# simonfuhrmann/mve

Measured on NVIDIA H100. Metric: mvs_depth_pixels_per_second, higher is better.
Workload: dtype f32

## Files before the change

### mve_b200/csrc/b200mvs.cu

```cuda
#include "../../include/b200mvs.h"
#include "patch_opt.cuh"
#include "patch_warp.cuh"
#include "patch_thread.cuh"
#include "pset_device.cuh"
#include "device_buffer.cuh"

#include <algorithm>
#include <cmath>
#include <cstdarg>
#include <cstddef>
#include <cstdio>
#include <cstring>
#include <cstdlib>
#include <functional>
#include <map>
#include <chrono>
#include <ctime>
#include <mutex>
#include <string>
#include <thread>
#include <atomic>
#include <vector>

using namespace b200mvs;
// ... 43 lines not shown

struct Entry {
    int xy;
    int jobdir;
    float conf, depth, dzI, dzJ;
    unsigned slots;
    int pad;
};
static_assert(sizeof(Entry) == 32, "Entry layout");

__host__ __device__ __forceinline__ int pack_xy(int x, int y) { return x | (y << 16); }
__host__ __device__ __forceinline__ Entry make_entry(int xy, int job, int dir, float conf, float depth, float dzI, float dzJ, unsigned slots)
{
    return Entry{xy, job | (dir << 24), conf, depth, dzI, dzJ, slots, 0};
}
__device__ __forceinline__ int entry_x(const Entry& e) { return e.xy & 0xFFFF; }
__device__ __forceinline__ int entry_y(const Entry& e) { return (e.xy >> 16) & 0xFFFF; }
__device__ __forceinline__ int entry_job(const Entry& e) { return e.jobdir & 0xFFFFFF; }
__device__ __forceinline__ int entry_dir(const Entry& e) { return (e.jobdir >> 24) & 7; }
__device__ __forceinline__ int pixel_of(const JobParams& J, const Entry& e) { return entry_y(e) * J.W + entry_x(e); }
__device__ __forceinline__ long long tile_of(const JobParams& J, const Entry& e) { return J.tile_base + (long long)(entry_y(e) >> 4) * J.tiles_x + (entry_x(e) >> 4); }
__device__ __forceinline__ Entry child_entry(int xy, int job, int dir, const PatchOut& r) { return make_entry(xy, job, dir, r.conf, r.depth, r.dzI, r.dzJ, r.slots); }
__device__ __forceinline__ unsigned long long seed_key(float c, size_t i) { return ((unsigned long long)__float_as_uint(c) << 32) | (0xFFFFFFFFu - (unsigned)i); }

enum Counter { C_RUN = 0, C_NEXT = 1, C_OVERFLOW = 2, C_SETS = 3, C_OPTS = 4, C_SEED_OK = 5, C_FILLED = 6, C_TICKET = 7, C_NUM = 8 };

constexpr int HIST_FINE = 8192;
constexpr int HIST_COARSE = 64;
constexpr int HIST_PER_JOB = HIST_FINE + HIST_COARSE;
constexpr int DEFER_BIT = 1 << 27;
enum Phase { PH_SEED = 0, PH_SELECT = 1, PH_THRESHOLD = 2, PH_PICK = 3, PH_OPT = 4, PH_COMMIT = 5, PH_EXPAND = 6, PH_SORT = 7, PH_OPT_THREAD = 8, PH_NUM = 9 };
enum Stop { ST_RUN = 0, ST_CANCELLED = 2, ST_OVERFLOW = 3, ST_GROW = 4 };

struct FrontierCtl {
    unsigned long long bar;
    unsigned long long nlist[2];
    unsigned long long nrun;
    unsigned long long ticket;
    unsigned long long ticket2;
    unsigned long long sort_cursor;
    unsigned long long small_cursor;
    unsigned long long rounds, peak, barriers;
    unsigned long long ns[PH_NUM];
    unsigned long long need;
    unsigned long long resume_ncur, resume_nrun;
    int resume_p, resume_sorted;
    int stop;
    int pad;
};

struct HostMirror {
    volatile int cancel;
    volatile int pad;
    volatile unsigned long long round, queue;
};

constexpr int MAX_GROUP_VIEWS = 4000;

struct HostCounters {
    unsigned long long count[C_NUM + MAX_GROUP_VIEWS];
    FrontierCtl ctl;
};
static_assert(offsetof(HostCounters, ctl) >= sizeof(unsigned long long) * (C_NUM + MAX_GROUP_VIEWS),
              "the counters of a full group end before the control block");

cudaError_t dev_alloc(b200mvs_ctx* ctx, void** p, size_t bytes);
void dev_free(b200mvs_ctx* ctx, void* p, size_t bytes);

template <typename T> struct DevBuf {
    T* p = nullptr;
    size_t cap = 0;
    cudaError_t reserve(b200mvs_ctx* ctx, size_t n)
    {
        if (n <= cap) return cudaSuccess;
// ... 505 lines not shown
}

__host__ __device__ inline int slots_to_ids(const int* gview, int n_global, unsigned word, int32_t ids[4])
{
    int n = 0;
#pragma unroll
    for (int k = 0; k < 4; ++k) {
        const unsigned sl = (word >> (8 * k)) & 0xFF;
        ids[k] = sl < (unsigned)n_global ? gview[sl] : -1;
        n += ids[k] >= 0;
    }
    return n;
}

__global__ void k_slots_to_ids(const JobParams job, int32_t* __restrict__ out, bool aligned16)
{
    const size_t p = (size_t)blockIdx.x * blockDim.x + threadIdx.x;
    if (p >= (size_t)job.W * job.H) return;
    int32_t ids[4];
    slots_to_ids(job.gview, job.n_global, __ldg(job.slots + p), ids);
    int32_t* o = out + 4 * p;
    if (aligned16) *reinterpret_cast<int4*>(o) = make_int4(ids[0], ids[1], ids[2], ids[3]);
    else { o[0] = ids[0]; o[1] = ids[1]; o[2] = ids[2]; o[3] = ids[3]; }
}

#ifndef OPT_MIN_BLOCKS
#define OPT_MIN_BLOCKS 1
#endif
constexpr int OPT_WARPS = OPT_TPB / 32;
using PatchT = b200mvs::PatchW;
using PatchT1 = b200mvs::PatchT;
constexpr size_t OPT_LUT_BYTES = sizeof(float) * (256 * LUT_STRIDE);
constexpr size_t OPT_SMEM_BYTES = OPT_LUT_BYTES + (size_t)OPT_TPB * sizeof(PatchT1) + PatchT1::MT_BYTES;
static_assert(OPT_SMEM_BYTES + 8 + 1024 <= 196 * 1024, "the patch kernels' shared memory must stay within the 196 KB carve-out");
__device__ __forceinline__ PatchT1& thread_patch(float* smem)
{
    return reinterpret_cast<PatchT1*>(reinterpret_cast<unsigned char*>(smem) + OPT_LUT_BYTES)[threadIdx.x];
}

__device__ __forceinline__ Entry load_entry(const Entry* p)
{
    const int4 a = __ldcg(reinterpret_cast<const int4*>(p));
    const int4 b = __ldcg(reinterpret_cast<const int4*>(p) + 1);
    Entry e;
    e.xy = a.x; e.jobdir = a.y; e.conf = __int_as_float(a.z); e.depth = __int_as_float(a.w);
    e.dzI = __int_as_float(b.x); e.dzJ = __int_as_float(b.y); e.slots = (unsigned)b.z; e.pad = b.w;
    return e;
}

__device__ __forceinline__ PatchIn patch_in(const Entry& e)
{
    PatchIn pi;
    pi.x = entry_x(e); pi.y = entry_y(e);
    pi.depth = e.depth; pi.dzI = e.dzI; pi.dzJ = e.dzJ; pi.slots = e.slots;
    return pi;
}

__device__ __forceinline__ unsigned long long global_timer_ns()
{
    unsigned long long t;
    asm volatile("mov.u64 %0, %%globaltimer;" : "=l"(t));
    return t;
}

__device__ __forceinline__ void optimise_entries(PatchT& p, const Entry* list, PatchOut* res, unsigned long long n,
                                                 unsigned long long* ticket, const JobParams* jobs, unsigned long long* counters)
{
// ... 34 lines not shown
            base = __shfl_sync(act, base, leader);
            const unsigned long long w = base + (unsigned long long)__popc(act & ((1u << lane) - 1u));
            if (w >= n) break;
            idx = w;
            const Entry e = load_entry(&list[w]);
            p.begin(&jobs[entry_job(e)], patch_in(e));
            have = true;
            ++opts;
        }
        if (p.step()) {
            PatchOut po;
            p.finish(po);
            res[idx] = po;
            have = false;
        }
    }
    if (opts) {
        atomicAdd(&counters[C_SETS], (unsigned long long)p.n_sets);
        atomicAdd(&counters[C_OPTS], (unsigned long long)opts);
        p.n_sets = 0u;
    }
}

#ifndef OPT_THREAD_MIN
#define OPT_THREAD_MIN 8192
#endif

__global__ void __launch_bounds__(OPT_TPB, OPT_MIN_BLOCKS)
k_optimize(const Entry* __restrict__ in, PatchOut* __restrict__ out, int n, int mode,
           const DevSettings* __restrict__ st, const JobParams* __restrict__ jobs, const ViewParams* __restrict__ views,
           const float* __restrict__ g_lut, unsigned long long* counters)
{
    extern __shared__ float smem[];
    for (int i = threadIdx.x; i < 256 * LUT_STRIDE; i += blockDim.x) smem[i] = g_lut[i / LUT_STRIDE];
    __syncthreads();
    if (mode == 2 || (mode == 0 && n >= OPT_THREAD_MIN)) {
        PatchT1& p = thread_patch(smem);
        bind_thread(p, st, views, smem, (int)threadIdx.x);
        optimise_entries_t(p, in, out, (unsigned long long)n, &counters[C_TICKET], jobs, counters);
    } else {
        PatchT p;
        bind_thread(p, st, views, smem, (int)threadIdx.x);
        optimise_entries(p, in, out, (unsigned long long)n, &counters[C_TICKET], jobs, counters);
    }
}

__device__ __forceinline__ unsigned long long entry_key(const Entry& e)
{
    return ((unsigned long long)__float_as_uint(e.conf) << 8) | (unsigned long long)(7 - entry_dir(e));
}

struct FrontierParams {
    Entry* list[2];
    Entry* run;
    Entry* run2;
    unsigned* tile_cnt;
    unsigned long long* tile_off;
    long long n_tiles;
    PatchOut* res;
    unsigned char* written;
    unsigned long long cap;
    int n_seeds, n_jobs;
    const DevSettings* st;
    const JobParams* jobs;
    const ViewParams* views;
    const float* lut;
    unsigned long long* counters;
    FrontierCtl* ctl;
    unsigned* hist;
    int* thr_bin;
    HostMirror* host;
    volatile unsigned long long* host_filled;
    volatile int* host_cancel_job;
    int* job_cancel;
    long long thread_min;
    unsigned long long* job_run;
    int band_bins;
    int topk;
    int first_list;
};

__device__ __forceinline__ unsigned long long ld_relaxed_u64(const unsigned long long* p)
{
    unsigned long long v;
    asm volatile("ld.relaxed.gpu.global.u64 %0, [%1];" : "=l"(v) : "l"(p) : "memory");
    return v;
}
__device__ __forceinline__ void grid_barrier(unsigned long long* bar)
{
    __syncthreads();
    if (threadIdx.x == 0) {
        __threadfence();
        const unsigned long long nb = gridDim.x;
        const unsigned long long t = atomicAdd(bar, 1ull);
        const unsigned long long target = (t / nb + 1ull) * nb;
        while (ld_relaxed_u64(bar) < target) __nanosleep(64);
        __threadfence();
    }
    __syncthreads();
}
__device__ __forceinline__ int conf_bin(float c)
{
    const int b = (int)(c * (float)HIST_FINE);
    return b < 0 ? 0 : (b > HIST_FINE - 1 ? HIST_FINE - 1 : b);
}
__device__ __forceinline__ PatchOut load_result(const PatchOut* p)
{
    static_assert(sizeof(PatchOut) == 40, "PatchOut layout");
    const int2* q = reinterpret_cast<const int2*>(p);
    const int2 a = __ldcg(q), b = __ldcg(q + 1), c = __ldcg(q + 2), d = __ldcg(q + 3), e = __ldcg(q + 4);
    PatchOut r;
    r.conf = __int_as_float(a.x); r.depth = __int_as_float(a.y); r.dzI = __int_as_float(b.x); r.dzJ = __int_as_float(b.y);
    r.nx = __int_as_float(c.x); r.ny = __int_as_float(c.y); r.nz = __int_as_float(d.x); r.slots = (unsigned)d.y;
    r.iterations = e.x; r.flags = e.y;
    return r;
}
__device__ __forceinline__ unsigned long long take_slot(unsigned long long* counter)
{
    const unsigned m = __activemask();
    const int lane = threadIdx.x & 31, leader = __ffs(m) - 1;
    unsigned long long base = 0ull;
    if (lane == leader) base = atomicAdd(counter, (unsigned long long)__popc(m));
    base = __shfl_sync(m, base, leader);
    return base + (unsigned long long)__popc(m & ((1u << lane) - 1u));
}
__device__ __forceinline__ void count_for_job(unsigned long long* per_job, int j)
{
    const unsigned m = __match_any_sync(__activemask(), j);
    if ((int)(threadIdx.x & 31) == __ffs(m) - 1) atomicAdd(&per_job[j], (unsigned long long)__popc(m));
}
__device__ __forceinline__ void push_entry(const FrontierParams& P, int q, const Entry& o)
{
    const unsigned long long pos = take_slot(&P.ctl->nlist[q]);
// ... 68 lines not shown
        const PatchOut r = load_result(&P.res[i]);
        const int j = entry_job(e);
        const JobParams& J = P.jobs[j];
        const int x = entry_x(e), y = entry_y(e);
        const int nx[4] = {x - 1, x + 1, x, x};
        const int ny[4] = {y, y, y - 1, y + 1};
#pragma unroll
        for (int d = 0; d < 4; ++d) {
            const float c = __ldcg(&J.conf[ny[d] * J.W + nx[d]]);
            if (c < r.conf - 0.05f || c == 0.f) push_entry(P, 1 - p, child_entry(pack_xy(nx[d], ny[d]), j, d, r));
        }
    }
}

__device__ __forceinline__ bool end_round(FrontierCtl* ctl, unsigned long long n_cur, const HostMirror* host)
{
    ctl->rounds += 1ull;
    if (n_cur > ctl->peak) ctl->peak = n_cur;
    return host->cancel != 0;
}

__global__ void k_frontier_resume(const FrontierParams P)
{
    FrontierCtl* const ctl = P.ctl;
    const size_t gtid = (size_t)blockIdx.x * blockDim.x + threadIdx.x, gthreads = (size_t)gridDim.x * blockDim.x;
    push_neighbours(P, ctl->resume_p, ctl->resume_sorted ? P.run2 : P.run, ctl->resume_nrun, gtid, gthreads);
    if (gtid == 0) ctl->stop = end_round(ctl, ctl->resume_ncur, P.host) ? ST_CANCELLED : ST_RUN;
}

__global__ void __launch_bounds__(OPT_TPB, OPT_MIN_BLOCKS)
k_frontier(const FrontierParams P)
{
    extern __shared__ float smem[];
    for (int i = threadIdx.x; i < 256 * LUT_STRIDE; i += blockDim.x) smem[i] = P.lut[i / LUT_STRIDE];
    __syncthreads();
    const int lane = threadIdx.x & 31;
    const size_t gtid = (size_t)blockIdx.x * blockDim.x + threadIdx.x, gthreads = (size_t)gridDim.x * blockDim.x;
    FrontierCtl* const ctl = P.ctl;
    unsigned long long* const cnt = P.counters;
    unsigned long long* const filled = cnt + C_NUM;
    const bool lead = blockIdx.x == 0 && threadIdx.x == 0;
    const bool thresholded = P.band_bins > 0 || P.topk > 0;
    unsigned long long t_prev = lead ? global_timer_ns() : 0ull;
    unsigned long long n_bar = 0ull;
#define PHASE_END(ph) do { grid_barrier(&ctl->bar); ++n_bar; if (lead) { const unsigned long long t_ = global_timer_ns(); ctl->ns[ph] += t_ - t_prev; t_prev = t_; } } while (0)

    int p = P.first_list;
    bool seed_round = P.n_seeds > 0;
    for (;;) {
        unsigned long long n_cur = seed_round ? (unsigned long long)P.n_seeds : __ldcg(&ctl->nlist[p]);
        if (n_cur > P.cap) n_cur = P.cap;
        if (__ldcg(&ctl->stop) != ST_RUN || n_cur == 0ull) break;
        unsigned long long n_run = n_cur;
        if (!seed_round) {
        Entry* const cur = P.list[p];
        if (blockIdx.x == 0) {
            if (threadIdx.x == 0) { P.host->round = ctl->rounds; P.host->queue = n_cur; }
            for (int j = threadIdx.x; j < P.n_jobs; j += blockDim.x) {
                P.host_filled[j] = __ldcg(&filled[j]);
                if (P.host_cancel_job[j]) P.job_cancel[j] = 1;
            }
        }
        for (size_t i = gtid; i < n_cur; i += gthreads) {
            const Entry e = load_entry(&cur[i]);
            const int j = entry_job(e);
            const JobParams& J = P.jobs[j];
            const int idx = pixel_of(J, e);
// ... 35 lines not shown
                count_for_job(P.job_run, entry_job(e));
            } else
                push_entry(P, 1 - p, e);
        }
        if (thresholded)
            for (size_t i = gtid; i < (size_t)P.n_jobs * HIST_PER_JOB; i += gthreads) P.hist[i] = 0u;
        PHASE_END(PH_PICK);
        n_run = __ldcg(&ctl->nrun);
        if (lead) { ctl->nlist[p] = 0ull; ctl->need = 0ull; }
        }
        unsigned long long n_thread = 0ull;
        const Entry* run_cur = P.run;
        if (!seed_round && P.n_tiles > 0) {
            __shared__ unsigned long long s_big;
            if (threadIdx.x == 0) s_big = 0ull;
            __syncthreads();
            unsigned long long mine = 0ull;
            for (int j = threadIdx.x; j < P.n_jobs; j += blockDim.x) {
                const unsigned long long c = __ldcg(&P.job_run[j]);
                if (c >= (unsigned long long)P.thread_min) mine += c;
            }
            if (mine) atomicAdd(&s_big, mine);
            __syncthreads();
            n_thread = s_big;
        }
        if (n_thread > 0ull) {
            for (size_t i = gtid; i < n_run; i += gthreads) {
                const Entry e = load_entry(&P.run[i]);
                const int j = entry_job(e);
                if (__ldcg(&P.job_run[j]) < (unsigned long long)P.thread_min) continue;
                atomicAdd(&P.tile_cnt[tile_of(P.jobs[j], e)], 1u);
            }
            PHASE_END(PH_SORT);
            for (size_t b = gtid; b < (size_t)P.n_tiles; b += gthreads) {
                const unsigned c = __ldcg(&P.tile_cnt[b]);
                if (c) P.tile_off[b] = atomicAdd(&ctl->sort_cursor, (unsigned long long)c);
            }
            PHASE_END(PH_SORT);
            for (size_t i = gtid; i < n_run; i += gthreads) {
                const Entry e = load_entry(&P.run[i]);
                const int j = entry_job(e);
                if (__ldcg(&P.job_run[j]) < (unsigned long long)P.thread_min) {
                    P.run2[n_thread + take_slot(&ctl->small_cursor)] = e;
                    continue;
                }
                const long long bin = tile_of(P.jobs[j], e);
                const unsigned k = atomicSub(&P.tile_cnt[bin], 1u) - 1u;
                P.run2[__ldcg(&P.tile_off[bin]) + k] = e;
            }
            PHASE_END(PH_SORT);
            run_cur = P.run2;
        }
        const bool by_thread = n_thread > 0ull;
        if (by_thread) {
            PatchT1& pt = thread_patch(smem);
            bind_thread(pt, P.st, P.views, smem, (int)threadIdx.x);
            optimise_entries_t(pt, run_cur, P.res, n_thread, &ctl->ticket, P.jobs, cnt);
            __syncwarp();
        }
        if (n_run > n_thread) {
            PatchT pg;
            bind_thread(pg, P.st, P.views, smem, (int)threadIdx.x);
            optimise_entries(pg, run_cur + n_thread, P.res + n_thread, n_run - n_thread, by_thread ? &ctl->ticket2 : &ctl->ticket, P.jobs, cnt);
        }
        if (seed_round) {
            PHASE_END(PH_SEED);
            for (size_t i = gtid; i < (size_t)P.n_seeds; i += gthreads) {
                const float c = __ldcg(&P.res[i].conf);
                if (!(c > 0.f)) continue;
// ... 11 lines not shown
                const JobParams& J = P.jobs[j];
                const int idx = pixel_of(J, e);
                if (__ldcg(&J.sel[idx]) != seed_key(c, i)) continue;
                J.sel[idx] = 0ull;
                count_for_job(filled, j);
                const PatchOut r = load_result(&P.res[i]);
                write_pixel(J, idx, r);
                push_entry(P, 0, child_entry(e.xy, j, 4, r));
            }
            if (lead) ctl->ticket = 0ull;
            PHASE_END(PH_COMMIT);
            seed_round = false;
            p = 0;
            continue;
        }
        if (by_thread) PHASE_END(PH_OPT_THREAD); else PHASE_END(PH_OPT);
        for (size_t i = gtid; i < n_run; i += gthreads) {
            const Entry e = load_entry(&run_cur[i]);
            const PatchOut r = load_result(&P.res[i]);
            const int j = entry_job(e);
            const JobParams& J = P.jobs[j];
            const int idx = pixel_of(J, e);
            unsigned char w = 0;
            if (!(r.conf == 0.f)) {
                const float old = __ldcg(&J.conf[idx]);
                if (old <= 0.f) count_for_job(filled, j);
                if (old < r.conf) { write_pixel(J, idx, r); w = 1; }
            }
            P.written[i] = w;
            const unsigned act = __activemask(), wm = __ballot_sync(act, w);
            if (wm && lane == __ffs(act) - 1) atomicAdd(&ctl->need, 4ull * (unsigned long long)__popc(wm));
        }
        if (lead) {
            ctl->nrun = 0ull; ctl->ticket = 0ull; ctl->ticket2 = 0ull; ctl->sort_cursor = 0ull; ctl->small_cursor = 0ull;
            atomicAdd(&ctl->need, __ldcg(&ctl->nlist[1 - p]));
        }
        if (blockIdx.x == 0) for (int j = threadIdx.x; j < P.n_jobs; j += blockDim.x) P.job_run[j] = 0ull;
        PHASE_END(PH_COMMIT);
        if (__ldcg(&ctl->need) > P.cap) {
            if (lead) {
                ctl->resume_p = p; ctl->resume_ncur = n_cur; ctl->resume_nrun = n_run; ctl->resume_sorted = run_cur == P.run2;
                ctl->stop = ST_GROW;
            }
            break;
        }
        push_neighbours(P, p, run_cur, n_run, gtid, gthreads);
        if (lead) {
            if (end_round(ctl, n_cur, P.host)) ctl->stop = ST_CANCELLED;
            else if (__ldcg(&cnt[C_OVERFLOW])) ctl->stop = ST_OVERFLOW;
        }
        PHASE_END(PH_EXPAND);
        p ^= 1;
    }
    if (lead) ctl->barriers += n_bar;
    if (blockIdx.x == 0) {
        if (threadIdx.x == 0) { P.host->round = ctl->rounds; P.host->queue = 0ull; }
        for (int j = threadIdx.x; j < P.n_jobs; j += blockDim.x) P.host_filled[j] = __ldcg(&filled[j]);
    }
#undef PHASE_END
}

int require_device(const b200mvs_ctx* ctx)
{
    return ctx->device != B200MVS_DEVICE_NONE ? 0 : fail(B200MVS_ERR_CUDA, "planning context (B200MVS_DEVICE_NONE): no CUDA device, b200mvs has no CPU fallback");
}

int check_camera_args(const b200mvs_ctx* ctx, const char* fn, int id, bool image, int w, int h, const float* pp, const float* rot, const float* trans)
// ... 116 lines not shown
    std::memset(hp.data(), 0, hp.size() * sizeof(ViewParams));
    for (size_t i = 0; i < ctx->views.size(); ++i) {
        const HostView& v = ctx->views[i];
        ViewParams& p = hp[i];
        p.valid = v.valid ? 1 : 0;
        if (!v.valid) continue;
        std::memcpy(p.campos, v.campos, 12);
        std::memcpy(p.w2c, v.w2c, 48);
        std::memcpy(p.rot, v.rot, 36);
        p.inv_ax0 = v.lv[0].invproj[0];
        p.nlevels = (int)v.lv.size();
        for (size_t l = 0; l < v.lv.size(); ++l) {
            const HostLevel& L = v.lv[l];
            p.lv[l].ax = L.proj[0]; p.lv[l].ay = L.proj[4]; p.lv[l].cx = L.proj[2]; p.lv[l].cy = L.proj[5];
            p.lv[l].w = L.w; p.lv[l].h = L.h; p.lv[l].pitch = L.pitch; p.lv[l].img = v.has_image ? L.d_img : nullptr;
            p.lv[l].quad = v.has_image ? L.d_quad : nullptr;
        }
    }
    CK(cudaMemcpyAsync(ctx->d_views, hp.data(), hp.size() * sizeof(ViewParams), cudaMemcpyHostToDevice, ctx->stream));
    CK(cudaStreamSynchronize(ctx->stream));
    ctx->views_dirty = false;
    return 0;
}

cudaEvent_t get_event(b200mvs_ctx* ctx, size_t i)
{
    while (ctx->ev_pool.size() <= i) { cudaEvent_t e; cudaEventCreate(&e); ctx->ev_pool.push_back(e); }
    return ctx->ev_pool[i];
}

int prepare_kernels(b200mvs_ctx* ctx)
{
    if (ctx->frontier_grid) return 0;
    CK(cudaFuncSetAttribute(k_frontier, cudaFuncAttributeMaxDynamicSharedMemorySize, (int)OPT_SMEM_BYTES));
    CK(cudaFuncSetAttribute(k_optimize, cudaFuncAttributeMaxDynamicSharedMemorySize, (int)OPT_SMEM_BYTES));
    int per_sm = 0, per_sm_opt = 0, sms = 0;
    CK(cudaOccupancyMaxActiveBlocksPerMultiprocessor(&per_sm, k_frontier, OPT_TPB, OPT_SMEM_BYTES));
    CK(cudaOccupancyMaxActiveBlocksPerMultiprocessor(&per_sm_opt, k_optimize, OPT_TPB, OPT_SMEM_BYTES));
    CK(cudaDeviceGetAttribute(&sms, cudaDevAttrMultiProcessorCount, ctx->device));
    if (per_sm < 1 || per_sm_opt < 1) return fail(B200MVS_ERR_CUDA, "patch-optimisation kernels do not fit on an SM");
    ctx->optimize_grid = per_sm_opt * sms;
    ctx->frontier_grid = per_sm * sms;
    return 0;
}

JobParams make_job(const b200mvs_ctx* ctx, const b200mvs_settings& s, int ref, const std::vector<int>& gsel)
{
    const HostLevel& L = ctx->views[ref].lv[s.scale];
    JobParams J;
    std::memset(&J, 0, sizeof(J));
    J.ref_view = ref; J.W = L.w; J.H = L.h; J.n_global = (int)gsel.size();
    for (size_t k = 0; k < gsel.size(); ++k) J.gview[k] = gsel[k];
    J.ki0 = L.invproj[0]; J.ki2 = L.invproj[2]; J.ki4 = L.invproj[4]; J.ki5 = L.invproj[5];
    J.ref_img = L.d_img; J.ref_pitch = L.pitch;
    return J;
}

unsigned ids_to_slots(const std::vector<int>& gsel, const int32_t* ids, int n, bool* ok)
{
    unsigned s = 0xFFFFFFFFu;
    std::vector<int> slots;
    for (int k = 0; k < n; ++k) {
        auto it = std::lower_bound(gsel.begin(), gsel.end(), (int)ids[k]);
        if (it == gsel.end() || *it != ids[k]) { *ok = false; return s; }
        slots.push_back((int)(it - gsel.begin()));
    }
    std::sort(slots.begin(), slots.end());
    for (size_t k = 0; k < slots.size() && k < 4; ++k) s = (s & ~(0xFFu << (8 * k))) | ((unsigned)slots[k] << (8 * k));
    *ok = true;
    return s;
}

int check_device_buffer(const char* fn, const std::string& what, const void* p, int device, size_t align)
// ... 1024 lines not shown
```

### mve_b200/csrc/patch_thread.cuh

```cuda
#pragma once
#include "patch_opt.cuh"
#if defined(B200MVS_HOST_EMU)
#include <cassert>
#endif

#ifndef OPT_TPB
#define OPT_TPB 384
#endif

namespace b200mvs {

struct alignas(8) SampleOffset { float di, dj; };
#if !defined(B200MVS_HOST_EMU)
__constant__
#endif
static const SampleOffset k_sample_offset[NS] = {
    {-2.f, -2.f}, {-1.f, -2.f}, {0.f, -2.f}, {1.f, -2.f}, {2.f, -2.f},
    {-2.f, -1.f}, {-1.f, -1.f}, {0.f, -1.f}, {1.f, -1.f}, {2.f, -1.f},
    {-2.f,  0.f}, {-1.f,  0.f}, {0.f,  0.f}, {1.f,  0.f}, {2.f,  0.f},
    {-2.f,  1.f}, {-1.f,  1.f}, {0.f,  1.f}, {1.f,  1.f}, {2.f,  1.f},
    {-2.f,  2.f}, {-1.f,  2.f}, {0.f,  2.f}, {1.f,  2.f}, {2.f,  2.f}};

struct PatchT : PatchState {
    const DevSettings* st;
// ... 23 lines not shown
    __device__ __forceinline__ int py() const { return (int)(xy >> 16); }

    template <typename T> static __device__ __forceinline__ T get4(const T (&a)[MAX_LOCAL], int k)
    {
        return k == 0 ? a[0] : (k == 1 ? a[1] : (k == 2 ? a[2] : a[3]));
    }
    template <typename T> static __device__ __forceinline__ void set4(T (&a)[MAX_LOCAL], int k, T v)
    {
#pragma unroll
        for (int i = 0; i < MAX_LOCAL; ++i) if (i == k) a[i] = v;
    }

    __device__ __forceinline__ unsigned lane_offset() const
    {
#if defined(B200MVS_HOST_EMU)
        return lane4;
#else
        return (threadIdx.x & 31u) << 2;
#endif
    }
    __device__ __forceinline__ const float* table() const
    {
#if defined(B200MVS_HOST_EMU)
        return lut_tab;
#else
        extern __shared__ float b200mvs_dyn_smem[];
        return b200mvs_dyn_smem;
#endif
    }

#if defined(B200MVS_HOST_EMU)
    static constexpr unsigned MT_STRIDE = 1u;
#else
    static constexpr unsigned MT_STRIDE = OPT_TPB;
#endif
    static constexpr size_t MT_BYTES = sizeof(unsigned) * NS * OPT_TPB;
    __device__ __forceinline__ unsigned* mt_tab()
    {
#if defined(B200MVS_HOST_EMU)
        return mt_k;
#else
        extern __shared__ float b200mvs_dyn_smem[];
        return reinterpret_cast<unsigned*>(b200mvs_dyn_smem + (256 * LUT_STRIDE + OPT_TPB * (sizeof(PatchT) / sizeof(float)))) + threadIdx.x;
#endif
    }

    __device__ __forceinline__ void sample_ray(float di, float dj, float& ux, float& uy, float& uz, float& inv) const
    {
        ux = u0x + di * uax + dj * ubx;
        uy = u0y + di * uay + dj * uby;
        uz = u0z + di * uaz + dj * ubz;
        inv = rsqrt_fast(ux * ux + uy * uy + uz * uz);
    }

    __device__ __forceinline__ void compute_points()
    {
        bool bad = false;
#pragma unroll 5
        for (int k = 0; k < NS; ++k) {
            const float t = depth + (float)(k % 5 - 2) * dzI + (float)(k / 5 - 2) * dzJ;
            bad |= t <= 0.f;
        }
        if (bad) pk &= ~F_REF_OK;
        cpx = c0x + depth * crx;
        cpy = c0y + depth * cry;
        cpz = c0z + depth * crz;
        const ViewParams* rv = &views[job->ref_view];
        const float z = __ldg(&rv->w2c[8]) * cpx + __ldg(&rv->w2c[9]) * cpy + __ldg(&rv->w2c[10]) * cpz + __ldg(&rv->w2c[11]);
        mfp = z * job->ki0;
        inv_mfp = rcp_fast(mfp);
    }

    __device__ __forceinline__ void init_sampler(int x, int y)
    {
        const float* const lut_tab = table();
        const unsigned lane4 = lane_offset();
// ... 28 lines not shown
            row += job->ref_pitch;
        }
        mm = (s0 + s1 + s2) / (3.f * NS);
        if (mm < 0.01f || mm > 0.99f) { pk &= ~F_REF_OK; return; }
        inv_mm = 1.f / mm;
        mx0 = (s0 * inv_mm) / (float)NS; mx1 = (s1 * inv_mm) / (float)NS; mx2 = (s2 * inv_mm) / (float)NS;
        float dev = 0.f;
#pragma unroll 1
        for (int j = 0; j < 5; ++j) {
#pragma unroll
            for (int i = 0; i < 5; ++i) {
                const unsigned t = mt[(5 * j + i) * MT_STRIDE];
                const float e0 = lut_k<0>(lut_tab, lane4, t) * inv_mm - mx0, e1 = lut_k<1>(lut_tab, lane4, t) * inv_mm - mx1, e2 = lut_k<2>(lut_tab, lane4, t) * inv_mm - mx2;
                dev += e0 * e0 + e1 * e1 + e2 * e2;
            }
        }
        sqrDevX = dev;
        compute_points();
    }

    struct Staged {
        uint4 Q;
        unsigned mt;
        float fx, fy, gx, gy;
    };
    struct Sweep {
        const float* lut;
        unsigned lane4;
        float inv_mm;
        float u0x, u0y, u0z, uax, uay, uaz, ubx, uby, ubz, depth, dzI, dzJ;
        const unsigned* mt;
        float A0x, A0y, A0z, W0x, W0y, W0z, Wax, Way, Waz, Wbx, Wby, Wbz;
        float Lax, Lay, Lcx, Lcy, wm1, hm1, step, dd;
        const uint4* quad;
        unsigned qpitch;
        float pv0, pv1, pv2;
        float c0, c1, c2;
        bool nrm;
        float Sya, Syb, Syc, Syya, Syyb, Syyc, Smya, Smyb, Smyc;
        float Sdma, Sdmb, Sdmc, Sdna, Sdnb, Sdnc, Sdda, Sddb, Sddc;
        float A1, A2, A3, A4, A5, B1, B2;

        __device__ __forceinline__ void clear()
        {
            Sya = Syb = Syc = Syya = Syyb = Syyc = Smya = Smyb = Smyc = 0.f;
            Sdma = Sdmb = Sdmc = Sdna = Sdnb = Sdnc = Sdda = Sddb = Sddc = 0.f;
            A1 = A2 = A3 = A4 = A5 = B1 = B2 = 0.f;
        }

        __device__ __forceinline__ bool stage(int k, Staged& s) const
        {
            const float di = k_sample_offset[k].di, dj = k_sample_offset[k].dj;
            const float ux = fma_rn(dj, ubx, fma_rn(di, uax, u0x)), uy = fma_rn(dj, uby, fma_rn(di, uay, u0y)), uz = fma_rn(dj, ubz, fma_rn(di, uaz, u0z));
            const float inv = rsqrt_fast(fma_rn(uz, uz, fma_rn(ux, ux, mul_rn(uy, uy))));
            const float s1 = mul_rn(fma_rn(dj, dzJ, fma_rn(di, dzI, depth)), inv);
            const float wx = fma_rn(dj, Wbx, fma_rn(di, Wax, W0x)), wy = fma_rn(dj, Wby, fma_rn(di, Way, W0y)), wz = fma_rn(dj, Wbz, fma_rn(di, Waz, W0z));
            const float hx = fma_rn(s1, wx, A0x), hy = fma_rn(s1, wy, A0y), hz = fma_rn(s1, wz, A0z);
            const float ih = rcp_fast(hz);
            const float qx = fma_rn(fma_rn(Lax, hx, mul_rn(Lcx, hz)), ih, -0.5f);
            const float qy = fma_rn(fma_rn(Lay, hy, mul_rn(Lcy, hz)), ih, -0.5f);
            const bool ok = qx > 0.f && qx < wm1 && qy > 0.f && qy < hm1;
            const float s2 = fma_rn(step, inv, s1);
            const float kx = fma_rn(s2, wx, A0x), ky = fma_rn(s2, wy, A0y), kz = fma_rn(s2, wz, A0z);
            const float ik = rcp_fast(kz);
            s.gx = sub_rn(fma_rn(fma_rn(Lax, kx, mul_rn(Lcx, kz)), ik, -0.5f), qx);
            s.gy = sub_rn(fma_rn(fma_rn(Lay, ky, mul_rn(Lcy, kz)), ik, -0.5f), qy);
            const float cx = ok ? qx : 0.f, cy = ok ? qy : 0.f;
            const int left = (int)floorf(cx), top = (int)floorf(cy);
#if defined(B200MVS_HOST_EMU)
            assert(left >= 0 && top >= 0 && (float)left < wm1 && (float)top < hm1);
#endif
            s.fx = sub_rn(cx, (float)left);
            s.fy = sub_rn(cy, (float)top);
            s.Q = __ldg(quad + ((unsigned)top * qpitch + (unsigned)left));
            s.mt = mt[k * MT_STRIDE];
            return ok;
        }

        __device__ __forceinline__ void sample(int k, const Staged& in)
        {
            const float fx = in.fx, fy = in.fy, gx = in.gx, gy = in.gy;
            const float m[3] = {mul_rn(lut_k<0>(lut, lane4, in.mt), inv_mm), mul_rn(lut_k<1>(lut, lane4, in.mt), inv_mm), mul_rn(lut_k<2>(lut, lane4, in.mt), inv_mm)};
            float a[3], b[3], c[3], e[3];
            a[0] = lut_k<0>(lut, lane4, in.Q.x); a[1] = lut_k<1>(lut, lane4, in.Q.x); a[2] = lut_k<2>(lut, lane4, in.Q.x);
            b[0] = lut_k<0>(lut, lane4, in.Q.y); b[1] = lut_k<1>(lut, lane4, in.Q.y); b[2] = lut_k<2>(lut, lane4, in.Q.y);
            c[0] = lut_k<0>(lut, lane4, in.Q.z); c[1] = lut_k<1>(lut, lane4, in.Q.z); c[2] = lut_k<2>(lut, lane4, in.Q.z);
            e[0] = lut_k<0>(lut, lane4, in.Q.w); e[1] = lut_k<1>(lut, lane4, in.Q.w); e[2] = lut_k<2>(lut, lane4, in.Q.w);
            const float omfx = sub_rn(1.f, fx), omfy = sub_rn(1.f, fy), wxy = fma_rn(fy, gx, mul_rn(fx, gy));
            float n[3], d[3];
#pragma unroll
            for (int ch = 0; ch < 3; ++ch) {
                const float x0 = fma_rn(omfx, a[ch], mul_rn(fx, b[ch]));
                const float x3 = fma_rn(omfx, c[ch], mul_rn(fx, e[ch]));
                n[ch] = fma_rn(omfy, x0, mul_rn(fy, x3));
                const float t = fma_rn(gx, sub_rn(b[ch], a[ch]), mul_rn(gy, sub_rn(c[ch], a[ch])));
                d[ch] = mul_rn(fma_rn(wxy, add_rn(sub_rn(sub_rn(a[ch], b[ch]), c[ch]), e[ch]), t), dd);
            }
            const float y0 = sub_rn(n[0], pv0), y1 = sub_rn(n[1], pv1), y2 = sub_rn(n[2], pv2);
            Sya = add_rn(Sya, y0); Syb = add_rn(Syb, y1); Syc = add_rn(Syc, y2);
            Syya = fma_rn(y0, y0, Syya); Syyb = fma_rn(y1, y1, Syyb); Syyc = fma_rn(y2, y2, Syyc);
            Smya = fma_rn(m[0], y0, Smya); Smyb = fma_rn(m[1], y1, Smyb); Smyc = fma_rn(m[2], y2, Smyc);
            Sdma = fma_rn(d[0], m[0], Sdma); Sdmb = fma_rn(d[1], m[1], Sdmb); Sdmc = fma_rn(d[2], m[2], Sdmc);
            Sdna = fma_rn(d[0], n[0], Sdna); Sdnb = fma_rn(d[1], n[1], Sdnb); Sdnc = fma_rn(d[2], n[2], Sdnc);
            Sdda = fma_rn(d[0], d[0], Sdda); Sddb = fma_rn(d[1], d[1], Sddb); Sddc = fma_rn(d[2], d[2], Sddc);
            if (nrm) {
                const float di = k_sample_offset[k].di, dj = k_sample_offset[k].dj;
                const float g0 = mul_rn(c0, d[0]), g1 = mul_rn(c1, d[1]), g2 = mul_rn(c2, d[2]);
// ... 8 lines not shown

    __device__ __forceinline__ void pass(bool candidates, bool cs_pending, bool want_ncc, bool want_normal, float* cand, PassOut& po)
    {
        const float* const lut_tab = table();
        const unsigned lane4 = lane_offset();
        const float u0x = this->u0x, u0y = this->u0y, u0z = this->u0z, uax = this->uax, uay = this->uay, uaz = this->uaz;
        const float ubx = this->ubx, uby = this->uby, ubz = this->ubz;
        const float depth = this->depth, dzI = this->dzI, dzJ = this->dzJ;
        const float inv_mm = this->inv_mm;
        const JobParams* const job = this->job;
        float num = 0.f, den = 0.f;
        double D0 = 0.0, D1 = 0.0, D2 = 0.0, D3 = 0.0, D4 = 0.0, D5 = 0.0, E0 = 0.0, E1 = 0.0, E2 = 0.0;
        bool cs_active = cs_pending && st->use_color_scale;
        if (!candidates) pk &= want_ncc ? ~((0xFFu << SH_COL) | (0xFu << SH_DF)) : ~(0xFFu << SH_COL);
        const int count = candidates ? job->n_global : nsel();
        const float pv0 = mx0 * mm, pv1 = mx1 * mm, pv2 = mx2 * mm;
#pragma unroll 1
        for (int k = 0; k < count; ++k) {
            int slot = k;
            if (candidates) { if (!((avail >> k) & 1u)) continue; }
            else slot = sel(k);
            const ViewParams* V = &views[job->gview[slot]];
            ++n_sets;
            float c0 = 1.f, c1 = 1.f, c2 = 1.f;
            if (!candidates) {
                c0 = k == 0 ? cs[0][0] : (k == 1 ? cs[1][0] : (k == 2 ? cs[2][0] : cs[3][0]));
                c1 = k == 0 ? cs[0][1] : (k == 1 ? cs[1][1] : (k == 2 ? cs[2][1] : cs[3][1]));
                c2 = k == 0 ? cs[0][2] : (k == 1 ? cs[1][2] : (k == 2 ? cs[2][2] : cs[3][2]));
            }
            unsigned r = 0u;
            float A0x = 0.f, A0y = 0.f, A0z = 0.f, W0x = 0.f, W0y = 0.f, W0z = 0.f, Wax = 0.f, Way = 0.f, Waz = 0.f, Wbx = 0.f, Wby = 0.f, Wbz = 0.f;
            float Lax = 0.f, Lay = 0.f, Lcx = 0.f, Lcy = 0.f, wm1 = 0.f, hm1 = 0.f, dd = 0.f, step = 0.f;
            int Lpitch = 0;
            const uint4* Lquad = nullptr;
            {
                const float4 wa = __ldg(reinterpret_cast<const float4*>(&V->w2c[0]));
                const float4 wb = __ldg(reinterpret_cast<const float4*>(&V->w2c[4]));
                const float4 wc = __ldg(reinterpret_cast<const float4*>(&V->w2c[8]));
                A0x = wa.x * c0x + wa.y * c0y + wa.z * c0z + wa.w;
                A0y = wb.x * c0x + wb.y * c0y + wb.z * c0z + wb.w;
                A0z = wc.x * c0x + wc.y * c0y + wc.z * c0z + wc.w;
                W0x = wa.x * u0x + wa.y * u0y + wa.z * u0z; W0y = wb.x * u0x + wb.y * u0y + wb.z * u0z; W0z = wc.x * u0x + wc.y * u0y + wc.z * u0z;
                Wax = wa.x * uax + wa.y * uay + wa.z * uaz; Way = wb.x * uax + wb.y * uay + wb.z * uaz; Waz = wc.x * uax + wc.y * uay + wc.z * uaz;
                Wbx = wa.x * ubx + wa.y * uby + wa.z * ubz; Wby = wb.x * ubx + wb.y * uby + wb.z * ubz; Wbz = wc.x * ubx + wc.y * uby + wc.z * ubz;
                const float nz = wc.x * cpx + wc.y * cpy + wc.z * cpz + wc.w;
                const float nfp = nz * __ldg(&V->inv_ax0);
                if (mfp > 0.f && !(nfp <= 0.f)) {
                    const int l = level_of(V, nfp, inv_mfp);
                    const float4 kk = __ldg(reinterpret_cast<const float4*>(&V->lv[l].ax));
                    const int4 g = __ldg(reinterpret_cast<const int4*>(&V->lv[l].w));
                    Lax = kk.x; Lay = kk.y; Lcx = kk.z; Lcy = kk.w; wm1 = (float)(g.x - 1); hm1 = (float)(g.y - 1); Lpitch = g.z;
                    Lquad = reinterpret_cast<const uint4*>(__ldg(reinterpret_cast<const unsigned long long*>(&V->lv[l].quad)));
                    const float inv0 = rsqrt_fast(u0x * u0x + u0y * u0y + u0z * u0z);
                    const float sa = depth * inv0, sb = (depth + 1.f) * inv0;
                    const float hz1 = A0z + sa * W0z, hz2 = A0z + sb * W0z;
                    const float i1 = rcp_fast(hz1), i2 = rcp_fast(hz2);
                    const float ddx = (Lax * (A0x + sb * W0x) + Lcx * hz2) * i2 - (Lax * (A0x + sa * W0x) + Lcx * hz1) * i1;
                    const float ddy = (Lay * (A0y + sb * W0y) + Lcy * hz2) * i2 - (Lay * (A0y + sa * W0y) + Lcy * hz1) * i1;
                    const float dd2 = ddx * ddx + ddy * ddy;
                    dd = dd2 * rsqrt_fast(dd2);
                    step = rcp_fast(dd);
                    r = dd > 0.f ? 3u : 1u;
                }
            }
            const bool need_ncc = candidates || want_ncc;
            const bool cs_view = !candidates && cs_active;
            float nccv = -1.f;
#pragma unroll 1
            for (int rep = 0; rep < 2 && r != 0u; ++rep) {
                const bool second = rep == 1;
                if (second && !(cs_view && want_normal && (r & 2u))) break;
                const bool gn = !candidates && (r & 2u) && (second || !(cs_view && want_normal));
                const bool nrm = gn && want_normal;
                Sweep sw;
                sw.lut = lut_tab; sw.lane4 = lane4; sw.inv_mm = inv_mm;
                sw.u0x = u0x; sw.u0y = u0y; sw.u0z = u0z; sw.uax = uax; sw.uay = uay; sw.uaz = uaz; sw.ubx = ubx; sw.uby = uby; sw.ubz = ubz;
                sw.mt = mt_tab();
                sw.depth = depth; sw.dzI = dzI; sw.dzJ = dzJ;
                sw.A0x = A0x; sw.A0y = A0y; sw.A0z = A0z; sw.W0x = W0x; sw.W0y = W0y; sw.W0z = W0z;
                sw.Wax = Wax; sw.Way = Way; sw.Waz = Waz; sw.Wbx = Wbx; sw.Wby = Wby; sw.Wbz = Wbz;
                sw.Lax = Lax; sw.Lay = Lay; sw.Lcx = Lcx; sw.Lcy = Lcy; sw.wm1 = wm1; sw.hm1 = hm1; sw.step = step; sw.dd = dd;
                sw.quad = Lquad; sw.qpitch = (unsigned)Lpitch;
                sw.pv0 = pv0; sw.pv1 = pv1; sw.pv2 = pv2; sw.c0 = c0; sw.c1 = c1; sw.c2 = c2; sw.nrm = nrm;
                sw.clear();
                Staged sa, sb;
                bool ok = sw.stage(0, sa);
                ok &= sw.stage(1, sb);
#pragma unroll 1
                for (int j = 0; j < NS - 3; j += 2) {
                    sw.sample(j, sa);
                    ok &= sw.stage(j + 2, sa);
                    sw.sample(j + 1, sb);
                    ok &= sw.stage(j + 3, sb);
                }
                sw.sample(NS - 3, sa);
                ok &= sw.stage(NS - 1, sa);
                sw.sample(NS - 2, sb);
                sw.sample(NS - 1, sa);
                const float Sya = sw.Sya, Syb = sw.Syb, Syc = sw.Syc, Syya = sw.Syya, Syyb = sw.Syyb, Syyc = sw.Syyc;
                const float Smya = sw.Smya, Smyb = sw.Smyb, Smyc = sw.Smyc, Sdma = sw.Sdma, Sdmb = sw.Sdmb, Sdmc = sw.Sdmc;
                const float Sdna = sw.Sdna, Sdnb = sw.Sdnb, Sdnc = sw.Sdnc, Sdda = sw.Sdda, Sddb = sw.Sddb, Sddc = sw.Sddc;
                const float A1 = sw.A1, A2 = sw.A2, A3 = sw.A3, A4 = sw.A4, A5 = sw.A5, B1 = sw.B1, B2 = sw.B2;
                if (!ok) { r = 0u; break; }
                if (!second && need_ncc) {
                    const float inv_n = 1.f / (float)NS;
                    const float sqrDevY = (Syya - Sya * Sya * inv_n) + (Syyb - Syb * Syb * inv_n) + (Syyc - Syc * Syc * inv_n);
                    const float Sen = (Smya - mx0 * Sya) + (Smyb - mx1 * Syb) + (Smyc - mx2 * Syc);
                    const float p = sqrDevX * sqrDevY;
                    nccv = p > 0.f ? Sen * rsqrt_fast(p) : -1.f;
                }
                if (!second && cs_view) {
                    const float Mna = Smya + pv0 * ((float)NS * mx0), Mnb = Smyb + pv1 * ((float)NS * mx1), Mnc = Smyc + pv2 * ((float)NS * mx2);
                    const float Nna = Syya + pv0 * (2.f * Sya + (float)NS * pv0), Nnb = Syyb + pv1 * (2.f * Syb + (float)NS * pv1);
                    const float Nnc = Syyc + pv2 * (2.f * Syc + (float)NS * pv2);
                    float cc[3] = {c0, c1, c2};
// ... 223 lines not shown
```

Baseline: 70.77 million.

## Pack per-warp mt tables into LUT padding and read images directly

The shared-memory LUT fill now writes only the LUT_REP replicated slots per row, and the per-thread mt scratch tables are packed into the unused padding of the LUT stride for some warps, with the rest in a smaller tail region. This shrinks the dynamic shared-memory footprint and sets an explicit carveout percentage so more L1 is left as cache. The bilinear sampler now loads four scalar texels from the plain image instead of one precomputed quad uint4. That trades one 16-byte load for four 4-byte loads but avoids the quad buffer's memory traffic. The new shared-memory indexing and carveout arithmetic add correctness and occupancy risk.

```diff
diff --git a/mve_b200/csrc/b200mvs.cu b/mve_b200/csrc/b200mvs.cu
--- a/mve_b200/csrc/b200mvs.cu
+++ b/mve_b200/csrc/b200mvs.cu
@@ -678,7 +678,13 @@
 using PatchT1 = b200mvs::PatchT;
 constexpr size_t OPT_LUT_BYTES = sizeof(float) * (256 * LUT_STRIDE);
 constexpr size_t OPT_SMEM_BYTES = OPT_LUT_BYTES + (size_t)OPT_TPB * sizeof(PatchT1) + PatchT1::MT_BYTES;
-static_assert(OPT_SMEM_BYTES + 8 + 1024 <= 196 * 1024, "the patch kernels' shared memory must stay within the 196 KB carve-out");
+constexpr size_t OPT_STATIC_SMEM_BYTES = 16;
+static_assert(OPT_SMEM_BYTES + OPT_STATIC_SMEM_BYTES + 1024 <= 164 * 1024, "the patch kernels' shared memory must stay within the 164 KB carve-out");
+
+__device__ __forceinline__ void fill_lut(float* smem, const float* lut)
+{
+    for (int i = threadIdx.x; i < 256 * LUT_REP; i += blockDim.x) smem[(i / LUT_REP) * LUT_STRIDE + i % LUT_REP] = lut[i / LUT_REP];
+}
 __device__ __forceinline__ PatchT1& thread_patch(float* smem)
 {
     return reinterpret_cast<PatchT1*>(reinterpret_cast<unsigned char*>(smem) + OPT_LUT_BYTES)[threadIdx.x];
@@ -779,7 +785,7 @@
            const float* __restrict__ g_lut, unsigned long long* counters)
 {
     extern __shared__ float smem[];
-    for (int i = threadIdx.x; i < 256 * LUT_STRIDE; i += blockDim.x) smem[i] = g_lut[i / LUT_STRIDE];
+    fill_lut(smem, g_lut);
     __syncthreads();
     if (mode == 2 || (mode == 0 && n >= OPT_THREAD_MIN)) {
         PatchT1& p = thread_patch(smem);
@@ -980,7 +986,7 @@
 k_frontier(const FrontierParams P)
 {
     extern __shared__ float smem[];
-    for (int i = threadIdx.x; i < 256 * LUT_STRIDE; i += blockDim.x) smem[i] = P.lut[i / LUT_STRIDE];
+    fill_lut(smem, P.lut);
     __syncthreads();
     const int lane = threadIdx.x & 31;
     const size_t gtid = (size_t)blockIdx.x * blockDim.x + threadIdx.x, gthreads = (size_t)gridDim.x * blockDim.x;
@@ -1345,8 +1351,17 @@
 int prepare_kernels(b200mvs_ctx* ctx)
 {
     if (ctx->frontier_grid) return 0;
-    CK(cudaFuncSetAttribute(k_frontier, cudaFuncAttributeMaxDynamicSharedMemorySize, (int)OPT_SMEM_BYTES));
-    CK(cudaFuncSetAttribute(k_optimize, cudaFuncAttributeMaxDynamicSharedMemorySize, (int)OPT_SMEM_BYTES));
+    int smem_sm = 0, reserved = 0;
+    CK(cudaDeviceGetAttribute(&smem_sm, cudaDevAttrMaxSharedMemoryPerMultiprocessor, ctx->device));
+    CK(cudaDeviceGetAttribute(&reserved, cudaDevAttrReservedSharedMemoryPerBlock, ctx->device));
+    for (const void* f : {(const void*)k_frontier, (const void*)k_optimize}) {
+        cudaFuncAttributes fa;
+        CK(cudaFuncGetAttributes(&fa, f));
+        const size_t need = (size_t)OPT_MIN_BLOCKS * (OPT_SMEM_BYTES + fa.sharedSizeBytes + (size_t)reserved);
+        const int pct = (int)std::min<size_t>(100, (100 * need + (size_t)smem_sm - 1) / (size_t)smem_sm);
+        CK(cudaFuncSetAttribute(f, cudaFuncAttributeMaxDynamicSharedMemorySize, (int)OPT_SMEM_BYTES));
+        CK(cudaFuncSetAttribute(f, cudaFuncAttributePreferredSharedMemoryCarveout, pct));
+    }
     int per_sm = 0, per_sm_opt = 0, sms = 0;
     CK(cudaOccupancyMaxActiveBlocksPerMultiprocessor(&per_sm, k_frontier, OPT_TPB, OPT_SMEM_BYTES));
     CK(cudaOccupancyMaxActiveBlocksPerMultiprocessor(&per_sm_opt, k_optimize, OPT_TPB, OPT_SMEM_BYTES));
diff --git a/mve_b200/csrc/patch_thread.cuh b/mve_b200/csrc/patch_thread.cuh
--- a/mve_b200/csrc/patch_thread.cuh
+++ b/mve_b200/csrc/patch_thread.cuh
@@ -79,16 +79,22 @@
 #if defined(B200MVS_HOST_EMU)
     static constexpr unsigned MT_STRIDE = 1u;
 #else
-    static constexpr unsigned MT_STRIDE = OPT_TPB;
-#endif
-    static constexpr size_t MT_BYTES = sizeof(unsigned) * NS * OPT_TPB;
+    static constexpr unsigned MT_STRIDE = LUT_STRIDE;
+#endif
+    static constexpr int MT_HOLE_WARPS = 256 / NS;
+    static constexpr int MT_BLOCK_WARPS = OPT_TPB / 32 > MT_HOLE_WARPS ? OPT_TPB / 32 - MT_HOLE_WARPS : 0;
+    static constexpr size_t MT_BYTES = sizeof(float) * LUT_STRIDE * NS * ((MT_BLOCK_WARPS + 1) / 2);
     __device__ __forceinline__ unsigned* mt_tab()
     {
 #if defined(B200MVS_HOST_EMU)
         return mt_k;
 #else
         extern __shared__ float b200mvs_dyn_smem[];
-        return reinterpret_cast<unsigned*>(b200mvs_dyn_smem + (256 * LUT_STRIDE + OPT_TPB * (sizeof(PatchT) / sizeof(float)))) + threadIdx.x;
+        const unsigned w = threadIdx.x >> 5, e = w - (unsigned)MT_HOLE_WARPS;
+        const unsigned word = w < (unsigned)MT_HOLE_WARPS
+            ? w * (NS * LUT_STRIDE) + LUT_REP
+            : (unsigned)(256 * LUT_STRIDE + OPT_TPB * (sizeof(PatchT) / sizeof(float))) + (e >> 1) * (NS * LUT_STRIDE) + (e & 1u) * LUT_REP;
+        return reinterpret_cast<unsigned*>(b200mvs_dyn_smem + word) + (threadIdx.x & 31u);
 #endif
     }
 
@@ -183,8 +189,8 @@
         const unsigned* mt;
         float A0x, A0y, A0z, W0x, W0y, W0z, Wax, Way, Waz, Wbx, Wby, Wbz;
         float Lax, Lay, Lcx, Lcy, wm1, hm1, step, dd;
-        const uint4* quad;
-        unsigned qpitch;
+        const unsigned* img;
+        unsigned pitch;
         float pv0, pv1, pv2;
         float c0, c1, c2;
         bool nrm;
@@ -223,7 +229,9 @@
 #endif
             s.fx = sub_rn(cx, (float)left);
             s.fy = sub_rn(cy, (float)top);
-            s.Q = __ldg(quad + ((unsigned)top * qpitch + (unsigned)left));
+            const unsigned* const r0 = img + ((unsigned)top * pitch + (unsigned)left);
+            const unsigned* const r1 = r0 + pitch;
+            s.Q.x = __ldg(r0); s.Q.y = __ldg(r0 + 1); s.Q.z = __ldg(r1); s.Q.w = __ldg(r1 + 1);
             s.mt = mt[k * MT_STRIDE];
             return ok;
         }
@@ -298,7 +306,7 @@
             float A0x = 0.f, A0y = 0.f, A0z = 0.f, W0x = 0.f, W0y = 0.f, W0z = 0.f, Wax = 0.f, Way = 0.f, Waz = 0.f, Wbx = 0.f, Wby = 0.f, Wbz = 0.f;
             float Lax = 0.f, Lay = 0.f, Lcx = 0.f, Lcy = 0.f, wm1 = 0.f, hm1 = 0.f, dd = 0.f, step = 0.f;
             int Lpitch = 0;
-            const uint4* Lquad = nullptr;
+            const unsigned* Limg = nullptr;
             {
                 const float4 wa = __ldg(reinterpret_cast<const float4*>(&V->w2c[0]));
                 const float4 wb = __ldg(reinterpret_cast<const float4*>(&V->w2c[4]));
@@ -316,7 +324,7 @@
                     const float4 kk = __ldg(reinterpret_cast<const float4*>(&V->lv[l].ax));
                     const int4 g = __ldg(reinterpret_cast<const int4*>(&V->lv[l].w));
                     Lax = kk.x; Lay = kk.y; Lcx = kk.z; Lcy = kk.w; wm1 = (float)(g.x - 1); hm1 = (float)(g.y - 1); Lpitch = g.z;
-                    Lquad = reinterpret_cast<const uint4*>(__ldg(reinterpret_cast<const unsigned long long*>(&V->lv[l].quad)));
+                    Limg = reinterpret_cast<const unsigned*>(__ldg(reinterpret_cast<const unsigned long long*>(&V->lv[l].img)));
                     const float inv0 = rsqrt_fast(u0x * u0x + u0y * u0y + u0z * u0z);
                     const float sa = depth * inv0, sb = (depth + 1.f) * inv0;
                     const float hz1 = A0z + sa * W0z, hz2 = A0z + sb * W0z;
@@ -346,7 +354,7 @@
                 sw.A0x = A0x; sw.A0y = A0y; sw.A0z = A0z; sw.W0x = W0x; sw.W0y = W0y; sw.W0z = W0z;
                 sw.Wax = Wax; sw.Way = Way; sw.Waz = Waz; sw.Wbx = Wbx; sw.Wby = Wby; sw.Wbz = Wbz;
                 sw.Lax = Lax; sw.Lay = Lay; sw.Lcx = Lcx; sw.Lcy = Lcy; sw.wm1 = wm1; sw.hm1 = hm1; sw.step = step; sw.dd = dd;
-                sw.quad = Lquad; sw.qpitch = (unsigned)Lpitch;
+                sw.img = Limg; sw.pitch = (unsigned)Lpitch;
                 sw.pv0 = pv0; sw.pv1 = pv1; sw.pv2 = pv2; sw.c0 = c0; sw.c1 = c1; sw.c2 = c2; sw.nrm = nrm;
                 sw.clear();
                 Staged sa, sb;
```

Result: faster. 76.17 million, median of 6 (+7.6%).

## Replace atomic tile-offset allocation with a deterministic grid-wide prefix scan

Applied to the files above, without the earlier changes.

Tile offsets for the thread-path sort were handed out by an atomicAdd on a single global cursor, which serialises on one address and gives a non-deterministic tile order. Each block now sums a contiguous range of tiles, does a block-level scan, and publishes its total to a per-block slot in the control block. After a grid barrier, every block scans its predecessors' totals to get exclusive offsets. This adds one extra grid barrier and caps the grid at 512 CTAs, but tiles come out in spatial order, which may improve locality in the later optimisation pass.

```diff
diff --git a/mve_b200/csrc/b200mvs.cu b/mve_b200/csrc/b200mvs.cu
--- a/mve_b200/csrc/b200mvs.cu
+++ b/mve_b200/csrc/b200mvs.cu
@@ -99,14 +99,16 @@
 enum Phase { PH_SEED = 0, PH_SELECT = 1, PH_THRESHOLD = 2, PH_PICK = 3, PH_OPT = 4, PH_COMMIT = 5, PH_EXPAND = 6, PH_SORT = 7, PH_OPT_THREAD = 8, PH_NUM = 9 };
 enum Stop { ST_RUN = 0, ST_CANCELLED = 2, ST_OVERFLOW = 3, ST_GROW = 4 };
 
+constexpr int MAX_GRID = 512;
+
 struct FrontierCtl {
     unsigned long long bar;
     unsigned long long nlist[2];
     unsigned long long nrun;
     unsigned long long ticket;
     unsigned long long ticket2;
-    unsigned long long sort_cursor;
     unsigned long long small_cursor;
+    unsigned long long tile_sum[MAX_GRID];
     unsigned long long rounds, peak, barriers;
     unsigned long long ns[PH_NUM];
     unsigned long long need;
@@ -678,7 +680,7 @@
 using PatchT1 = b200mvs::PatchT;
 constexpr size_t OPT_LUT_BYTES = sizeof(float) * (256 * LUT_STRIDE);
 constexpr size_t OPT_SMEM_BYTES = OPT_LUT_BYTES + (size_t)OPT_TPB * sizeof(PatchT1) + PatchT1::MT_BYTES;
-static_assert(OPT_SMEM_BYTES + 8 + 1024 <= 196 * 1024, "the patch kernels' shared memory must stay within the 196 KB carve-out");
+static_assert(OPT_SMEM_BYTES + 112 + 1024 <= 196 * 1024, "the patch kernels' shared memory must stay within the 196 KB carve-out");
 __device__ __forceinline__ PatchT1& thread_patch(float* smem)
 {
     return reinterpret_cast<PatchT1*>(reinterpret_cast<unsigned char*>(smem) + OPT_LUT_BYTES)[threadIdx.x];
@@ -846,6 +848,25 @@
     }
     __syncthreads();
 }
+__device__ __forceinline__ unsigned long long block_scan(unsigned long long v, unsigned long long* total)
+{
+    __shared__ unsigned long long s_warp[OPT_WARPS];
+    const int lane = threadIdx.x & 31, warp = threadIdx.x >> 5;
+    unsigned long long incl = v;
+#pragma unroll
+    for (int o = 1; o < 32; o <<= 1) { const unsigned long long u = __shfl_up_sync(FULL, incl, o); if (lane >= o) incl += u; }
+    __syncthreads();
+    if (lane == 31) s_warp[warp] = incl;
+    __syncthreads();
+    unsigned long long before = 0ull, sum = 0ull;
+    for (int w = 0; w < OPT_WARPS; ++w) {
+        const unsigned long long s = s_warp[w];
+        if (w < warp) before += s;
+        sum += s;
+    }
+    *total = sum;
+    return before + incl - v;
+}
 __device__ __forceinline__ int conf_bin(float c)
 {
     const int b = (int)(c * (float)HIST_FINE);
@@ -1082,9 +1103,22 @@
                 atomicAdd(&P.tile_cnt[tile_of(P.jobs[j], e)], 1u);
             }
             PHASE_END(PH_SORT);
-            for (size_t b = gtid; b < (size_t)P.n_tiles; b += gthreads) {
+            const unsigned long long t_lo = (unsigned long long)P.n_tiles * blockIdx.x / gridDim.x;
+            const unsigned long long t_hi = (unsigned long long)P.n_tiles * (blockIdx.x + 1) / gridDim.x;
+            const unsigned long long t_a = t_lo + (t_hi - t_lo) * threadIdx.x / blockDim.x;
+            const unsigned long long t_b = t_lo + (t_hi - t_lo) * (threadIdx.x + 1) / blockDim.x;
+            unsigned long long mine = 0ull, total = 0ull, before = 0ull;
+            for (unsigned long long b = t_a; b < t_b; ++b) mine += __ldcg(&P.tile_cnt[b]);
+            unsigned long long off = block_scan(mine, &total);
+            if (threadIdx.x == 0) ctl->tile_sum[blockIdx.x] = total;
+            PHASE_END(PH_SORT);
+            for (unsigned b = threadIdx.x; b < blockIdx.x; b += blockDim.x) before += __ldcg(&ctl->tile_sum[b]);
+            block_scan(before, &total);
+            off += total;
+            for (unsigned long long b = t_a; b < t_b; ++b) {
                 const unsigned c = __ldcg(&P.tile_cnt[b]);
-                if (c) P.tile_off[b] = atomicAdd(&ctl->sort_cursor, (unsigned long long)c);
+                P.tile_off[b] = off;
+                off += c;
             }
             PHASE_END(PH_SORT);
             for (size_t i = gtid; i < n_run; i += gthreads) {
@@ -1162,7 +1196,7 @@
             if (wm && lane == __ffs(act) - 1) atomicAdd(&ctl->need, 4ull * (unsigned long long)__popc(wm));
         }
         if (lead) {
-            ctl->nrun = 0ull; ctl->ticket = 0ull; ctl->ticket2 = 0ull; ctl->sort_cursor = 0ull; ctl->small_cursor = 0ull;
+            ctl->nrun = 0ull; ctl->ticket = 0ull; ctl->ticket2 = 0ull; ctl->small_cursor = 0ull;
             atomicAdd(&ctl->need, __ldcg(&ctl->nlist[1 - p]));
         }
         if (blockIdx.x == 0) for (int j = threadIdx.x; j < P.n_jobs; j += blockDim.x) P.job_run[j] = 0ull;
@@ -1352,6 +1386,9 @@
     CK(cudaOccupancyMaxActiveBlocksPerMultiprocessor(&per_sm_opt, k_optimize, OPT_TPB, OPT_SMEM_BYTES));
     CK(cudaDeviceGetAttribute(&sms, cudaDevAttrMultiProcessorCount, ctx->device));
     if (per_sm < 1 || per_sm_opt < 1) return fail(B200MVS_ERR_CUDA, "patch-optimisation kernels do not fit on an SM");
+    if (per_sm * sms > MAX_GRID)
+        return fail(B200MVS_ERR_UNSUPPORTED, "%d SMs x %d CTAs: more than the %d CTAs of the frontier kernel's control block",
+                    sms, per_sm, MAX_GRID);
     ctx->optimize_grid = per_sm_opt * sms;
     ctx->frontier_grid = per_sm * sms;
     return 0;
```

New measurement: 70.62 million before, 71.86 million after (median of 6 runs). 1.02x the previous value.
